# aubin-tchoi/shot-fpfh

Measured on AMD Instinct MI355X. Metric: descriptors/sec (SHOT+FPFH) on 1M-pt cloud, higher is better.
Workload: dtype f64

## Files before the change

### shot_fpfh_amd/csrc/match.h

```cpp
#pragma once
#include <algorithm>
#include <cmath>
#include <cstdlib>
#include <functional>

#include "common.h"

int sf_match_exact(sf_ctx *ctx, const double *da, int64_t m1, const double *db, int64_t m2, int64_t d, int64_t *didx,
                   double *ddist, const char *name, const unsigned char *a_ok, const unsigned char *b_ok);
int sf_match_gemm(sf_ctx *ctx, const double *da, int64_t m1, const double *db, int64_t m2, int64_t d, int64_t *didx,
                  double *ddist, const char *name, int64_t *n_slow, const unsigned char *a_ok, const unsigned char *b_ok);
int sf_match_sqnorm(sf_ctx *ctx, const char *name, const double *rows, int64_t m, int64_t d, const unsigned char *ok, double *out);
int sf_match_gemm_f64(sf_ctx *ctx, const double *da, int64_t m1, const double *db, int64_t m2, int64_t d, int64_t *didx,
                      double *ddist, const char *name, int64_t *n_slow, const unsigned char *a_ok, const unsigned char *b_ok);
int sf_match_half_mode();
int sf_match_half(sf_ctx *ctx, const double *da, int64_t m1, const double *db, int64_t m2, int64_t d, int64_t *didx,
                  double *ddist, const char *name, int64_t *n_slow, const unsigned char *a_ok, const unsigned char *b_ok,
                  int *used);
int sf_match_i8_mode();
int sf_match_i8(sf_ctx *ctx, const double *da, int64_t m1, const double *db, int64_t m2, int64_t d, int64_t *didx,
                double *ddist, const char *name, int64_t *n_slow, const unsigned char *a_ok, const unsigned char *b_ok,
                int *used);

typedef std::function<int(const double *sub, int64_t nr, int64_t *sidx, double *sdist)> sf_match_next;
int sf_match_rescue(sf_ctx *ctx, const double *da, int64_t m1, int64_t d, const int *flag, int nf, const sf_match_next &next,
                    int64_t *didx, double *ddist, int64_t *n_slow, int per_row = 1, const char *gather_name = "k8_gather_rows",
                    const char *scatter_name = "k8_scatter_results");
int sf_match_max(sf_ctx *ctx, const char *name, const double *v, int64_t n, double *part, double *out);

static inline void sf_ransac_band(double thr, double *lo, double *hi)
{
    *lo = *hi = -1.0;
    if (thr >= 0.0) {
        const double up = std::nextafter(thr, INFINITY);
        *lo = std::nextafter(thr * thr, -INFINITY);
        *hi = std::isinf(up) ? INFINITY : std::nextafter(up * up, INFINITY);
        if (std::isinf(thr)) *lo = *hi = INFINITY;
    }
}

static inline bool sf_match_small(int64_t m1, int64_t m2, int64_t d)
{
    return (double)m1 * (double)m2 * (double)d < 5e8 || m2 < 256;
}

static inline int64_t sf_match_col_splits(int64_t row_tiles, int64_t col_tiles, int64_t target, int64_t *tiles_per_split)
{
    int64_t nsplit = 1;
    if (row_tiles < target) nsplit = std::min<int64_t>(col_tiles, sf_div_up(target, row_tiles));
    if (nsplit > 65535) nsplit = 65535;
    *tiles_per_split = sf_div_up(col_tiles, nsplit);
    return sf_div_up(col_tiles, *tiles_per_split);
}

static inline int64_t sf_match_splits(int64_t col_tiles, int64_t tile_bytes, int64_t row_blocks, const char *env)
{
    const int64_t chunk_kb = 8192;
    const int64_t tiles_in_l2 = std::max<int64_t>(8, chunk_kb * 1024 / tile_bytes);
    int64_t nsplit = sf_div_up(col_tiles, tiles_in_l2);
    if (row_blocks * nsplit < 512) nsplit = std::max<int64_t>(nsplit, std::min<int64_t>(sf_div_up(512, row_blocks), std::max<int64_t>(col_tiles / 32, 1)));
    if (const char *e = getenv(env)) nsplit = std::max<int64_t>(1, std::min<int64_t>(atoll(e), col_tiles));
    return nsplit;
}

template <int CTRL>
__device__ __forceinline__ int sf_dpp(int v)
{
    return __builtin_amdgcn_update_dpp(0, v, CTRL, 0xf, 0xf, false);
}
template <int CTRL>
__device__ __forceinline__ float sf_dpp(float v)
{
    return __int_as_float(sf_dpp<CTRL>(__float_as_int(v)));
}
template <int CTRL>
__device__ __forceinline__ double sf_dpp(double v)
{
    return __hiloint2double(sf_dpp<CTRL>(__double2hiint(v)), sf_dpp<CTRL>(__double2loint(v)));
}

__device__ __forceinline__ double sf_match_tol(int64_t d, double na, double nb_max)
{
    return 8.0 * (double)d * 1.1102230246251565e-16 * (na + nb_max);
}

struct sf_recheck {
    double best = INFINITY;
    int64_t bj = -1;
    bool ok = true;
};

__device__ __forceinline__ void sf_recheck_candidate(sf_recheck &r, const double *ai, const double *b, int64_t d, int64_t j,
                                                     double key, double na, double unit, double half_w)
{
    const double *bjp = b + j * d;
    double acc = 0.0;
    for (int64_t u = 0; u < d; ++u) {
        const double df = ai[u] - bjp[u];
        acc += df * df;
    }
    r.ok &= fabs((acc - na) * unit - key) <= half_w;
    const double dj = sqrt(acc);
    if (dj < r.best || (dj == r.best && j < r.bj) || r.bj < 0) {
        if (!(dj == dj)) return;
        r.best = dj;
        r.bj = j;
    }
}

template <int LPR>
__device__ __forceinline__ void sf_recheck_fold(sf_recheck &r)
{
#pragma unroll
    for (int off = LPR / 2; off > 0; off >>= 1) {
        const double ob = __shfl_xor(r.best, off);
        const int64_t oj = __shfl_xor(r.bj, off);
        const int om = __shfl_xor((int)r.ok, off);
        if (oj >= 0 && (r.bj < 0 || ob < r.best || (ob == r.best && oj < r.bj))) {
            r.best = ob;
            r.bj = oj;
        }
        r.ok = r.ok && om;
    }
}
```

### shot_fpfh_amd/csrc/match_half.hip

```cpp
#include <algorithm>
#include <cmath>
#include <cstdlib>

#include "device_util.h"
#include "match.h"

namespace {

typedef _Float16 h8 __attribute__((ext_vector_type(8)));
typedef float f16v __attribute__((ext_vector_type(16)));

constexpr int HM = 256;
constexpr int HN = 64;
constexpr int HCAP = 32;

__global__ __launch_bounds__(256) void k_half_convert(const double *__restrict__ a, int64_t m, int64_t m_pad, int64_t d,
                                                      int dp, double scale, const unsigned char *__restrict__ ok,
                                                      _Float16 *__restrict__ out, double *__restrict__ err,
                                                      double *__restrict__ qn, double *__restrict__ n2,
                                                      float *__restrict__ n2f, double n2f_scale)
{
    const int lane = threadIdx.x & 63;
    const int64_t i = (int64_t)blockIdx.x * 4 + (threadIdx.x >> 6);
    if (i >= m_pad) return;
// ... 154 lines not shown
        f16v acc[2];
        acc[0] = cold ? zero : T;
        acc[1] = acc[0];
#pragma unroll
        for (int ks = 0; ks < KS; ++ks) {
            acc[0] = __builtin_amdgcn_mfma_f32_32x32x16_f16(af[ks], q0[ks % PF], acc[0], 0, 0, 0);
            acc[1] = __builtin_amdgcn_mfma_f32_32x32x16_f16(af[ks], q1[ks % PF], acc[1], 0, 0, 0);
            if (ks + PF < KS) {
                q0[ks % PF] = SF_H_FRAG(ks + PF, 0);
                q1[ks % PF] = SF_H_FRAG(ks + PF, 1);
            }
        }
        __builtin_amdgcn_sched_group_barrier(0x100, 2 * PF, 0);
#pragma unroll
        for (int ks = 0; ks < KS; ++ks) {
            __builtin_amdgcn_sched_group_barrier(0x008, 2, 0);
            if (ks + PF < KS) __builtin_amdgcn_sched_group_barrier(0x100, 2, 0);
        }
        const float *nbl = reinterpret_cast<const float *>(bp + HN * PC * 16);
        const float nbv2[2] = {nbl[r31], nbl[32 + r31]};
#pragma unroll
        for (int cb = 0; cb < 2; ++cb) {
            const int64_t j = jt * HN + 32 * cb + r31;
            const float nbv = nbv2[cb];
            float mx = acc[cb][0];
#pragma unroll
            for (int r = 1; r < 16; ++r) mx = fmaxf(mx, acc[cb][r]);
            if (cold || __ballot(mx >= nbv)) {
                const bool was_cold = cold;
                int rowb = (int)(row0 - rb * HM) + 4 * h;
                asm volatile("" : "+v"(rowb));
                const int64_t rowbase = rb * HM + rowb;
#pragma unroll
                for (int r = 0; r < 16; ++r) {
                    const float dot = was_cold ? acc[cb][r] : acc[cb][r] - T[r];
                    const float key = nbv - dot;
                    const bool hit = (key <= T[r]) & (key < INFINITY);
                    if (__ballot(hit)) {
                        float v = hit ? key : INFINITY;
                        v = fminf(v, sf_dpp<0xB1>(v));
                        v = fminf(v, sf_dpp<0x4E>(v));
                        v = fminf(v, sf_dpp<0x141>(v));
                        v = fminf(v, sf_dpp<0x140>(v));
                        v = fminf(v, __shfl_xor(v, 16));
                        const int64_t row = rowbase + (r & 3) + 8 * (r >> 2);
                        const float tn = fminf(T[r], v + win[row]);
                        if (hit && key <= tn) {
                            const int s = atomicAdd(&cnt[row], 1);
                            if (s < HCAP) {
                                cand_j[row * HCAP + s] = (int32_t)j;
                                cand_k[row * HCAP + s] = key;
                            }
                        }
                        if (cb == 0 && !was_cold) acc[1][r] += tn - T[r];
                        T[r] = tn;
                    }
                }
                if (was_cold && cb == 1) {
                    bool c = false;
#pragma unroll
                    for (int r = 0; r < 16; ++r) c |= T[r] == INFINITY;
                    cold = __ballot(c) != 0;
                }
            }
        }
        asm volatile("s_waitcnt vmcnt(0)" ::: "memory");
        __syncthreads();
    }
    if (r31 == 0) {
#pragma unroll
        for (int r = 0; r < 16; ++r) {
            const int64_t row = row0 + (r & 3) + 8 * (r >> 2) + 4 * h;
            thr_out[row] = T[r];
            if (thr_best && row < m1 && T[r] < INFINITY) atomic_min_f32(thr_best + row, T[r]);
        }
    }
#undef SF_H_DMA
#undef SF_H_DMA16
#undef SF_H_DMA4
#undef SF_H_FRAG
}

template <int LPR>
__global__ void k_half_final(const double *__restrict__ a, int64_t m1, const double *__restrict__ b, int64_t d,
                             const unsigned char *__restrict__ a_ok, const int *__restrict__ cnt,
                             const int32_t *__restrict__ cand_j, const float *__restrict__ cand_k,
                             const float *__restrict__ thr, const float *__restrict__ win,
                             const double *__restrict__ na2, double unit, int nsplit, int64_t m1_pad,
                             int64_t *__restrict__ idx,
                             double *__restrict__ dist, int *__restrict__ flag, int *__restrict__ n_flagged)
{
    const int64_t gid = (int64_t)blockIdx.x * blockDim.x + threadIdx.x;
    const int64_t i = gid / LPR;
    const int sub = (int)(gid % LPR);
    if (i >= m1) return;
    if (a_ok && !a_ok[i]) {
        if (sub == 0) {
            idx[i] = 0;
            if (dist) dist[i] = INFINITY;
            flag[i] = 0;
        }
        return;
    }
    float t = INFINITY;
    for (int s = 0; s < nsplit; ++s) t = fminf(t, thr[(int64_t)s * m1_pad + i]);
    bool overflow = false;
    const float w = win[i] * 1.001f;
    for (int s = 0; s < nsplit; ++s)
        overflow |= cnt[(int64_t)s * m1_pad + i] > HCAP && !(thr[(int64_t)s * m1_pad + i] - w > t);
    sf_recheck r;
    if (!overflow) {
        const double *ai = a + i * d;
        const double half_w = 0.5 * (double)win[i], na = na2[i];
        for (int s = 0; s < nsplit; ++s) {
            const int64_t base = ((int64_t)s * m1_pad + i) * HCAP;
            const int n = min(cnt[(int64_t)s * m1_pad + i], HCAP);
            for (int c = sub; c < n; c += LPR)
                if (cand_k[base + c] <= t)
                    sf_recheck_candidate(r, ai, b, d, cand_j[base + c], (double)cand_k[base + c], na, unit, half_w);
        }
    }
    sf_recheck_fold<LPR>(r);
    if (sub != 0) return;
    const bool decided = r.bj >= 0 && r.ok;
    idx[i] = decided ? r.bj : 0;
    if (dist) dist[i] = r.best;
    flag[i] = decided ? 0 : 1;
    if (!decided) atomicAdd(n_flagged, 1);
}

bool pick_scale(double n2max, double *scale)
{
    if (!(n2max > 0.0) || !std::isfinite(n2max)) return false;
    int e = 0;
    std::frexp(std::sqrt(n2max), &e);
    const int k = 14 - e;
    if (k < -100 || k > 100) return false;
    *scale = std::ldexp(1.0, k);
    return true;
}

}

int sf_match_half_mode()
{
    const char *e = getenv("SF_MATCH_HALF");
    if (!e || !e[0]) return -1;
    return e[0] == '0' ? 0 : 1;
}

int sf_match_half(sf_ctx *ctx, const double *da, int64_t m1, const double *db, int64_t m2, int64_t d, int64_t *didx,
                  double *ddist, const char *name, int64_t *n_slow, const unsigned char *a_ok, const unsigned char *b_ok,
                  int *used)
{
    *used = 0;
    if (d > 352 || m1 <= 0 || m2 <= 0 || m2 > 0x7fffffff) return SF_OK;
    const int ks = d <= 128 ? 8 : 22, dp = 16 * ks;
    const int64_t m1p = sf_div_up(m1, HM) * HM, m2p = sf_div_up(m2, HN) * HN;
    _Float16 *ah = nullptr, *bh = nullptr;
    double *ea = nullptr, *qa = nullptr, *na2 = nullptr, *eb = nullptr, *qb = nullptr, *nb2 = nullptr, *part = nullptr;
    float *nbf = nullptr, *win = nullptr, *candk = nullptr, *thr = nullptr;
    int *cnt = nullptr, *flag = nullptr, *nflag = nullptr;
    int32_t *candj = nullptr;
    sf_pool_guard tmp(ctx);
#define SF_HALLOC(ptr, count) SF_CHECK(tmp.alloc(&ptr, (size_t)(count)))
    SF_HALLOC(part, 256);
    SF_HALLOC(nb2, m2p); SF_HALLOC(eb, m2p); SF_HALLOC(qb, m2p); SF_HALLOC(nbf, m2p);
    SF_HALLOC(na2, m1p); SF_HALLOC(ea, m1p); SF_HALLOC(qa, m1p);
    SF_HALLOC(ah, m1p * dp); SF_HALLOC(bh, m2p * dp);
    double namax = 0.0, nbmax = 0.0, sa = 1.0, sb = 1.0;
    {
        SF_LAUNCH(ctx, "k8_half_convert", k_half_convert, dim3((unsigned)sf_div_up(m1p, 4)), dim3(256), da, m1, m1p, d, dp,
                  1.0, (const unsigned char *)nullptr, (_Float16 *)nullptr, ea, qa, na2, (float *)nullptr, 1.0);
        SF_LAUNCH(ctx, "k8_half_convert", k_half_convert, dim3((unsigned)sf_div_up(m2p, 4)), dim3(256), db, m2, m2p, d, dp,
                  1.0, b_ok, (_Float16 *)nullptr, eb, qb, nb2, (float *)nullptr, 1.0);
        int rc = sf_match_max(ctx, "k8_half_max", na2, m1, part, &namax);
        if (rc == SF_OK) rc = sf_match_max(ctx, "k8_half_max", nb2, m2, part, &nbmax);
        if (rc != SF_OK) return rc;
    }
    if (!pick_scale(namax, &sa) || !pick_scale(nbmax, &sb)) return SF_OK;
    const double unit = 0.5 * sa * sb;
    if (!(nbmax * unit < 1e30) || !(nbmax * unit > 1e-20)) return SF_OK;
    SF_LAUNCH(ctx, "k8_half_convert", k_half_convert, dim3((unsigned)sf_div_up(m1p, 4)), dim3(256), da, m1, m1p, d, dp, sa,
              (const unsigned char *)nullptr, ah, ea, qa, na2, (float *)nullptr, 1.0);
    SF_LAUNCH(ctx, "k8_half_convert", k_half_convert, dim3((unsigned)sf_div_up(m2p, 4)), dim3(256), db, m2, m2p, d, dp, sb,
              b_ok, bh, eb, qb, nb2, nbf, unit);
    double ebmax = 0.0, qbmax = 0.0;
    {
        int rc = sf_match_max(ctx, "k8_half_max", eb, m2, part, &ebmax);
        if (rc == SF_OK) rc = sf_match_max(ctx, "k8_half_max", qb, m2, part, &qbmax);
        if (rc != SF_OK) return rc;
    }
    if (!std::isfinite(ebmax) || !std::isfinite(qbmax)) return SF_OK;
    const int64_t col_tiles = m2p / HN;
    int64_t nsplit = sf_match_splits(col_tiles, (int64_t)HN * dp * 2, m1p / HM, "SF_MATCH_HALF_SPLITS");
    const int64_t tiles_per_split = sf_div_up(col_tiles, nsplit);
    nsplit = sf_div_up(col_tiles, tiles_per_split);
    const bool seed = true;
    const int64_t slab_rows = std::min<int64_t>(m1p, HM * std::max<int64_t>(64, ((int64_t)8 << 30) / (nsplit * HCAP * 8 * HM)));
    float *tbest = nullptr;
    SF_HALLOC(win, slab_rows); SF_HALLOC(thr, nsplit * slab_rows); SF_HALLOC(cnt, nsplit * slab_rows); SF_HALLOC(tbest, slab_rows);
    SF_HALLOC(candj, nsplit * slab_rows * HCAP); SF_HALLOC(candk, nsplit * slab_rows * HCAP);
    SF_HALLOC(flag, m1); SF_HALLOC(nflag, 1);
    const double gamma = (double)(dp + 32) * 2.384185791015625e-07;
    SF_HIP(hipMemsetAsync(nflag, 0, sizeof(int), ctx->stream));
    for (int64_t r0 = 0; r0 < m1; r0 += slab_rows) {
        const int64_t ms = std::min(m1 - r0, slab_rows), msp = sf_div_up(ms, HM) * HM, row_blocks = msp / HM;
        SF_LAUNCH(ctx, "k8_half_window", k_half_window, dim3((unsigned)sf_div_up(msp, 256)), dim3(256), (const double *)(ea + r0),
                  (const double *)(qa + r0), (const double *)(na2 + r0), ms, msp, std::sqrt(nbmax), ebmax, qbmax, nbmax, gamma, unit, win);
        SF_HIP(hipMemsetAsync(cnt, 0, (size_t)(nsplit * msp) * sizeof(int), ctx->stream));
        SF_HIP(hipMemsetD32Async((hipDeviceptr_t)tbest, 0x7f800000, (size_t)msp, ctx->stream));
        const int64_t wgs = sf_xcd_grid(nsplit * row_blocks);
        if (wgs > 0x7fffffffLL) { sf_set_error("sf_match_half: %lld workgroups exceed a launch", (long long)wgs); return SF_ERR_UNSUPPORTED; }
        if (ks == 8) {
            SF_LAUNCH(ctx, name, k_match_half<8>, dim3((unsigned)wgs), dim3(512), (const _Float16 *)(ah + r0 * dp),
                      ms, (const _Float16 *)bh, m2p, (const float *)nbf, (const float *)win, tiles_per_split, msp, row_blocks, nsplit,
                      seed ? tbest : (float *)nullptr, cnt, candj, candk, thr);
        } else {
            SF_LAUNCH(ctx, name, k_match_half<22>, dim3((unsigned)wgs), dim3(512), (const _Float16 *)(ah + r0 * dp),
                      ms, (const _Float16 *)bh, m2p, (const float *)nbf, (const float *)win, tiles_per_split, msp, row_blocks, nsplit,
                      seed ? tbest : (float *)nullptr, cnt, candj, candk, thr);
        }
#define SF_HALF_FINAL(LPR)                                                                                            \
        SF_LAUNCH(ctx, "k8_half_final", k_half_final<LPR>, dim3((unsigned)sf_div_up(ms * LPR, 256)), dim3(256), da + r0 * d, ms, db, d, \
                  a_ok ? a_ok + r0 : a_ok, (const int *)cnt, (const int32_t *)candj, (const float *)candk, (const float *)thr, \
                  (const float *)win, (const double *)(na2 + r0), unit, (int)nsplit, msp, didx + r0, ddist ? ddist + r0 : ddist, \
                  flag + r0, nflag);
        const int lpr = ms <= 160000 ? 16 : 1;
        if (lpr == 1) { SF_HALF_FINAL(1) } else { SF_HALF_FINAL(16) }
#undef SF_HALF_FINAL
    }
    int nf = 0;
    SF_HIP(hipMemcpyAsync(&nf, nflag, sizeof(int), hipMemcpyDeviceToHost, ctx->stream));
    SF_HIP(hipStreamSynchronize(ctx->stream));
    const int rc = sf_match_rescue(ctx, da, m1, d, flag, nf, [&](const double *sub, int64_t nr, int64_t *sidx, double *sdist) {
        return sf_match_gemm_f64(ctx, sub, nr, db, m2, d, sidx, sdist, "k8_match_gemm_overflow", nullptr, nullptr, b_ok);
    }, didx, ddist, n_slow);
#undef SF_HALLOC
    *used = 1;
    return rc;
}
```

### shot_fpfh_amd/csrc/match_i8.hip

```cpp
#include <algorithm>
#include <cmath>
#include <cstdlib>
#include <vector>

#include "device_util.h"
#include "match.h"

namespace {

typedef int i4v __attribute__((ext_vector_type(4)));
typedef int i16v __attribute__((ext_vector_type(16)));

constexpr int IN = 64;
constexpr int ICAP = 32;
constexpr int I_LIVE = 4;
constexpr int I_BIG = 1 << 30;
constexpr int I_REAL = 1 << 29;

__global__ __launch_bounds__(256) void k_i8_rowstat(const double *__restrict__ a, int64_t m, int64_t d, double *__restrict__ n2,
                                                    double *__restrict__ amax)
{
    const int lane = threadIdx.x & 63;
    const int64_t i = (int64_t)blockIdx.x * 4 + (threadIdx.x >> 6);
    if (i >= m) return;
// ... 281 lines not shown
    }
}

template <int KS>
__global__ __launch_bounds__(512, 1) void k_i8_collect(const unsigned char *__restrict__ ai, const unsigned char *__restrict__ bi,
                                                        const int *__restrict__ nbs, const int2 *__restrict__ split_tiles,
                                                        int64_t n_blocks, const int *__restrict__ blk_split,
                                                        const int *__restrict__ pair_row, const int *__restrict__ pair_thr,
                                                        int *__restrict__ cnt, int32_t *__restrict__ cand_j,
                                                        int *__restrict__ cand_k)
{
    const int64_t vb = sf_xcd_block();
    if (vb >= n_blocks) return;
    const int64_t split = blk_split[vb];
    SF_I_GEOMETRY
    const int64_t p0 = vb * 256 + 32 * wave;
    i4v af[KS];
    {
        const int row = pair_row[p0 + r31];
        const unsigned char *ap = ai + (int64_t)(row < 0 ? 0 : row) * DP + 16 * h;
#pragma unroll
        for (int ks = 0; ks < KS; ++ks) af[ks] = *reinterpret_cast<const i4v *>(ap + 32 * ks);
#pragma unroll
        for (int ks = 0; ks < KS; ++ks) asm volatile("" : "+v"(af[ks]));
    }
    i16v T;
#pragma unroll
    for (int r = 0; r < 16; ++r) {
        const int64_t p = p0 + (r & 3) + 8 * (r >> 2) + 4 * h;
        T[r] = pair_row[p] < 0 ? -I_BIG : pair_thr[p];
    }
    const int2 st = split_tiles[split];
    const int64_t jt0 = st.x, ntiles = st.y;
    SF_I_DMA(jt0, 0)
    asm volatile("s_waitcnt vmcnt(0)" ::: "memory");
    __syncthreads();
    for (int64_t jt = jt0; jt < ntiles; ++jt) {
        const int buf = (int)((jt - jt0) & 1);
        if (jt + 1 < ntiles) SF_I_DMA(jt + 1, buf ^ 1)
        const unsigned char *bp = Bs + buf * TILE_BYTES;
        constexpr int PF = 3;
        const int *nbl = reinterpret_cast<const int *>(bp + IN * PC * 16);
#pragma unroll 1
        for (int cb = 0; cb < 2; ++cb) {
            i4v q[PF];
#pragma unroll
            for (int i = 0; i < PF; ++i) q[i] = SF_I_FRAG(i, cb);
            i16v acc = T;
#pragma unroll
            for (int ks = 0; ks < KS; ++ks) {
                acc = __builtin_amdgcn_mfma_i32_32x32x32_i8(af[ks], q[ks % PF], acc, 0, 0, 0);
                if (ks + PF < KS) q[ks % PF] = SF_I_FRAG(ks + PF, cb);
            }
            const int nbv = nbl[32 * cb + r31];
            int mx = acc[0];
#pragma unroll
            for (int r = 1; r < 16; ++r) mx = max(mx, acc[r]);
            if (__ballot(mx >= nbv && nbv < I_REAL)) {
                const int64_t j = jt * IN + 32 * cb + r31;
#pragma unroll
                for (int r = 0; r < 16; ++r) {
                    if (acc[r] >= nbv && nbv < I_REAL) {
                        const int64_t p = p0 + (r & 3) + 8 * (r >> 2) + 4 * h;
                        const int s = atomicAdd(&cnt[p], 1);
                        if (s < ICAP) {
                            cand_j[p * ICAP + s] = (int32_t)j;
                            cand_k[p * ICAP + s] = nbv - (acc[r] - T[r]);
                        }
                    }
                }
            }
        }
        asm volatile("s_waitcnt vmcnt(0)" ::: "memory");
        __syncthreads();
    }
}
#undef SF_I_DMA
#undef SF_I_DMA16
#undef SF_I_DMA4
#undef SF_I_FRAG
#undef SF_I_GEOMETRY

template <int LPR>
__global__ void k_i8_final(const double *__restrict__ a, int64_t m1, const double *__restrict__ b, int64_t d,
                           const unsigned char *__restrict__ a_ok, const int *__restrict__ live, const int *__restrict__ cnt,
                           const int32_t *__restrict__ cand_j, const int *__restrict__ cand_k, const int *__restrict__ win,
                           const double *__restrict__ na2, double unit, int64_t *__restrict__ idx, double *__restrict__ dist,
                           int *__restrict__ flag, int *__restrict__ n_flagged)
{
    const int64_t gid = (int64_t)blockIdx.x * blockDim.x + threadIdx.x;
    const int64_t i = gid / LPR;
    const int sub = (int)(gid % LPR);
    if (i >= m1) return;
    if ((a_ok && !a_ok[i]) || flag[i]) return;
    sf_recheck r;
    const double *ai = a + i * d;
    const double half_w = 0.5 * (double)win[i], na = na2[i];
    for (int l = 0; l < I_LIVE; ++l) {
        const int p = live[i * I_LIVE + l];
        if (p < 0) continue;
        const int n = cnt[p];
        if (n > ICAP) { r.ok = false; continue; }
        const int64_t base = (int64_t)p * ICAP;
        for (int c = sub; c < n; c += LPR)
            sf_recheck_candidate(r, ai, b, d, cand_j[base + c], (double)cand_k[base + c], na, unit, half_w);
    }
    sf_recheck_fold<LPR>(r);
    if (sub != 0) return;
    const bool decided = r.bj >= 0 && r.ok;
    idx[i] = decided ? r.bj : 0;
    if (dist) dist[i] = r.best;
    if (!decided) {
        flag[i] = 1;
        atomicAdd(n_flagged, 1);
    }
}

}

int sf_match_i8_mode()
{
    const char *e = getenv("SF_MATCH_I8");
    if (!e || !e[0]) return -1;
    return e[0] == '0' ? 0 : 1;
}

struct sf_match_stream {
    sf_ctx *ctx = nullptr;
    const double *da = nullptr, *db = nullptr;
    const unsigned char *a_ok = nullptr, *b_ok = nullptr;
    int64_t m1 = 0, m2 = 0, d = 0, m1p = 0, m2p = 0;
    int ks = 11, dp = 352, RB = 2, IM = 512;
    double sa = 0.0, sb = 0.0, unit = 0.0;
    bool integer = false;
    bool windowed = false;
    unsigned char *ai = nullptr, *bi = nullptr;
    double *ea = nullptr, *qa = nullptr, *na2 = nullptr, *eb = nullptr, *qb = nullptr, *nb2 = nullptr, *part = nullptr, *amx = nullptr;
    int *nbi = nullptr, *win = nullptr, *smin = nullptr, *kmin = nullptr, *live = nullptr, *flag = nullptr, *counters = nullptr;
    int2 *split_tiles = nullptr;
    int64_t split_cap = 0, tiles_target = 0;
    std::vector<int2> splits;
    std::vector<void *> owned;
    double nbmax = 0.0, ebmax = 0.0;
};

namespace {

template <typename T>
int st_alloc(sf_match_stream *st, T **p, size_t count)
{
    SF_CHECK(sf_palloc(st->ctx, p, count ? count : 1));
    st->owned.push_back(*p);
    return SF_OK;
}

void st_free(sf_match_stream *st)
{
    if (!st) return;
    for (void *p : st->owned) sf_pool_release(st->ctx, p);
    delete st;
}

int st_begin(sf_match_stream *st, double b_entry_max, int64_t max_ranges, bool *suitable)
{
    sf_ctx *ctx = st->ctx;
    *suitable = false;
    const int64_t m1 = st->m1, m2 = st->m2, d = st->d;
    if (d > 352 || m1 <= 0 || m2 <= 0 || m2 > 0x7fffffff || m1 > 0x3fffffff) return SF_OK;
    st->RB = 2;
    st->IM = 256 * st->RB;
    st->ks = d <= 128 ? 4 : 11;
    st->dp = 32 * st->ks;
    st->m1p = sf_div_up(m1, 512) * 512;
    st->m2p = sf_div_up(m2, IN) * IN;
    const int64_t m1p = st->m1p, m2p = st->m2p;
    SF_CHECK(st_alloc(st, &st->part, 256));
    SF_CHECK(st_alloc(st, &st->na2, m1p)); SF_CHECK(st_alloc(st, &st->ea, m1p)); SF_CHECK(st_alloc(st, &st->qa, m1p));
    SF_CHECK(st_alloc(st, &st->amx, std::max(m1, m2)));
    double namax = 0.0, aamax = 0.0;
    SF_LAUNCH(ctx, "k8_i8_convert", k_i8_rowstat, dim3((unsigned)sf_div_up(m1, 4)), dim3(256), st->da, m1, d, st->na2, st->amx);
    SF_CHECK(sf_match_max(ctx, "k8_i8_max", st->na2, m1, st->part, &namax));
    SF_CHECK(sf_match_max(ctx, "k8_i8_max", st->amx, m1, st->part, &aamax));
    if (!(aamax > 0.0) || !(b_entry_max > 0.0) || !std::isfinite(namax) || !std::isfinite(aamax) || !std::isfinite(b_entry_max)) return SF_OK;
    st->sa = 127.0 / aamax;
    st->sb = 127.0 / b_entry_max;
    st->unit = 0.5 * st->sa * st->sb;
    if (!std::isfinite(st->sa) || !std::isfinite(st->sb) || !std::isfinite(st->unit) || !(st->unit > 0.0)) return SF_OK;
    SF_CHECK(st_alloc(st, &st->ai, m1p * st->dp)); SF_CHECK(st_alloc(st, &st->bi, m2p * st->dp));
    SF_CHECK(st_alloc(st, &st->nb2, m2p)); SF_CHECK(st_alloc(st, &st->eb, m2p)); SF_CHECK(st_alloc(st, &st->qb, m2p)); SF_CHECK(st_alloc(st, &st->nbi, m2p));
    if (m1p > m1) SF_HIP(hipMemsetAsync(st->na2 + m1, 0, (size_t)(m1p - m1) * sizeof(double), ctx->stream));
    SF_LAUNCH(ctx, "k8_i8_convert", k_i8_convert, dim3((unsigned)sf_div_up(m1p, 4)), dim3(256), st->da, m1, m1p, d, st->dp, st->sa,
              (const unsigned char *)nullptr, reinterpret_cast<unsigned *>(st->ai), st->ea, st->qa, (const double *)st->na2, (int *)nullptr, st->unit);
    const int64_t col_tiles = m2p / IN;
    const int64_t nsplit = sf_match_splits(col_tiles, (int64_t)IN * st->dp, m1p / st->IM, "SF_MATCH_I8_SPLITS");
    st->tiles_target = sf_div_up(col_tiles, nsplit);
    st->split_cap = sf_div_up(col_tiles, st->tiles_target) + std::max<int64_t>(max_ranges, 1);
    if (st->split_cap > 65536) return SF_OK;
    SF_CHECK(st_alloc(st, &st->win, m1p)); SF_CHECK(st_alloc(st, &st->smin, st->split_cap * m1p)); SF_CHECK(st_alloc(st, &st->kmin, m1p));
    SF_CHECK(st_alloc(st, &st->live, m1p * I_LIVE)); SF_CHECK(st_alloc(st, &st->flag, m1));
    SF_CHECK(st_alloc(st, &st->counters, 2 * st->split_cap + 2));
    SF_CHECK(st_alloc(st, &st->split_tiles, st->split_cap));
    SF_HIP(hipMemsetAsync(st->counters, 0, (size_t)(2 * st->split_cap + 2) * sizeof(int), ctx->stream));
    *suitable = true;
    st->integer = true;
    return SF_OK;
}

int st_convert_cols(sf_match_stream *st, int64_t rb, int64_t re, int64_t *first, int64_t *count)
{
    sf_ctx *ctx = st->ctx;
    const int64_t rows = re - rb, rows_p = sf_div_up(rows, IN) * IN;
    if (rb % IN || rows <= 0 || re > st->m2 || (re % IN && re != st->m2)) { sf_set_error("sf_match_stream_feed: rows [%lld, %lld) are not whole 64-row tiles", (long long)rb, (long long)re); return SF_ERR_ARG; }
    SF_LAUNCH(ctx, "k8_i8_convert", k_i8_rowstat, dim3((unsigned)sf_div_up(rows, 4)), dim3(256), st->db + rb * st->d, rows, st->d, st->nb2 + rb, st->amx);
    if (rows_p > rows) SF_HIP(hipMemsetAsync(st->nb2 + re, 0, (size_t)(rows_p - rows) * sizeof(double), ctx->stream));
    SF_LAUNCH(ctx, "k8_i8_convert", k_i8_convert, dim3((unsigned)sf_div_up(rows_p, 4)), dim3(256), st->db + rb * st->d, rows, rows_p, st->d, st->dp, st->sb,
              st->b_ok ? st->b_ok + rb : st->b_ok, reinterpret_cast<unsigned *>(st->bi + rb * st->dp), st->eb + rb, st->qb + rb,
              (const double *)(st->nb2 + rb), st->nbi + rb, st->unit);
    const int64_t t0 = rb / IN, t1 = t0 + rows_p / IN, n = sf_div_up(t1 - t0, st->tiles_target), per = sf_div_up(t1 - t0, n);
    *first = (int64_t)st->splits.size();
    for (int64_t t = t0; t < t1; t += per) st->splits.push_back(make_int2((int)t, (int)std::min(t + per, t1)));
    *count = (int64_t)st->splits.size() - *first;
    if ((int64_t)st->splits.size() > st->split_cap) { sf_set_error("sf_match_stream_feed: more ranges than announced"); return SF_ERR_ARG; }
    SF_HIP(hipMemcpyAsync(st->split_tiles + *first, st->splits.data() + *first, (size_t)*count * sizeof(int2), hipMemcpyHostToDevice, ctx->stream));
    SF_HIP(hipStreamSynchronize(ctx->stream));
    return SF_OK;
}

int st_pass1(sf_match_stream *st, const char *name, int64_t first, int64_t count, int64_t r0, int64_t ms)
{
    sf_ctx *ctx = st->ctx;
    const int64_t msp = sf_div_up(ms, st->IM) * st->IM, row_blocks = msp / st->IM;
    const int64_t wgs = sf_xcd_grid(count * row_blocks);
    if (wgs > 0x7fffffffLL) { sf_set_error("sf_match_i8: %lld workgroups exceed a launch", (long long)wgs); return SF_ERR_UNSUPPORTED; }
    if (!count || !ms) return SF_OK;
#define SF_I8_MIN(KS_, RB_)                                                                                             \
    SF_LAUNCH(ctx, name, (k_i8_min<KS_, RB_>), dim3((unsigned)wgs), dim3(512), (const unsigned char *)(st->ai + r0 * st->dp), \
              (const unsigned char *)st->bi, (const int *)st->nbi, (const int2 *)st->split_tiles, first, st->m1p, row_blocks, count, st->smin + r0)
    if (st->ks == 4) { SF_I8_MIN(4, 2); } else { SF_I8_MIN(11, 2); }
#undef SF_I8_MIN
    return SF_OK;
}

int st_window(sf_match_stream *st, bool *suitable)
{
    sf_ctx *ctx = st->ctx;
    *suitable = false;
    SF_CHECK(sf_match_max(ctx, "k8_i8_max", st->nb2, st->m2, st->part, &st->nbmax));
    SF_CHECK(sf_match_max(ctx, "k8_i8_max", st->eb, st->m2, st->part, &st->ebmax));
    if (!std::isfinite(st->nbmax) || !std::isfinite(st->ebmax) || !(st->nbmax * st->unit < 4e6)) return SF_OK;
    SF_LAUNCH(ctx, "k8_i8_window", k_i8_window, dim3((unsigned)sf_div_up(st->m1p, 256)), dim3(256), (const double *)st->ea, (const double *)st->qa,
              (const double *)st->na2, st->m1, st->m1p, std::sqrt(st->nbmax), st->ebmax, st->nbmax, st->unit, st->win);
    st->windowed = true;
    *suitable = true;
    return SF_OK;
}

int st_decide(sf_match_stream *st, int64_t r0, int64_t ms, int64_t *didx, double *ddist)
{
    sf_ctx *ctx = st->ctx;
    const int64_t nsplit = (int64_t)st->splits.size(), m1p = st->m1p;
    int *nflag = st->counters, *split_count = st->counters + 2, *split_cursor = st->counters + 2 + st->split_cap;
    SF_HIP(hipMemsetAsync(split_count, 0, (size_t)(2 * st->split_cap) * sizeof(int), ctx->stream));
    SF_LAUNCH(ctx, "k8_i8_live", k_i8_live, dim3((unsigned)sf_div_up(ms, 256)), dim3(256), (const int *)(st->smin + r0), (const int *)(st->win + r0),
              st->a_ok ? st->a_ok + r0 : st->a_ok, ms, m1p, (int)nsplit, st->kmin + r0, st->live + r0 * I_LIVE, split_count, didx + r0,
              ddist ? ddist + r0 : ddist, st->flag + r0, nflag);
    std::vector<int> hcount((size_t)nsplit), hbase((size_t)nsplit), hblk;
    SF_HIP(hipMemcpyAsync(hcount.data(), split_count, (size_t)nsplit * sizeof(int), hipMemcpyDeviceToHost, ctx->stream));
    SF_HIP(hipStreamSynchronize(ctx->stream));
    int64_t n_pairs_pad = 0;
    for (int64_t s = 0; s < nsplit; ++s) {
        hbase[(size_t)s] = (int)n_pairs_pad;
        const int64_t nb = sf_div_up(hcount[(size_t)s], 256);
        for (int64_t k = 0; k < nb; ++k) hblk.push_back((int)s);
        n_pairs_pad += nb * 256;
        if (n_pairs_pad > 0x7fffff00LL) { sf_set_error("sf_match_i8: too many (row, split) pairs"); return SF_ERR_UNSUPPORTED; }
    }
    const int64_t n_blocks = (int64_t)hblk.size();
    sf_pool_guard ptmp(ctx);
    int *split_base = nullptr, *blk_split = nullptr, *pair_row = nullptr, *pair_thr = nullptr, *cnt = nullptr, *candk = nullptr;
    int32_t *candj = nullptr;
    const size_t np1 = (size_t)std::max<int64_t>(n_pairs_pad, 1);
    SF_CHECK(ptmp.alloc(&split_base, (size_t)nsplit)); SF_CHECK(ptmp.alloc(&blk_split, (size_t)std::max<int64_t>(n_blocks, 1)));
    SF_CHECK(ptmp.alloc(&pair_row, np1)); SF_CHECK(ptmp.alloc(&pair_thr, np1)); SF_CHECK(ptmp.alloc(&cnt, np1));
    SF_CHECK(ptmp.alloc(&candj, np1 * ICAP)); SF_CHECK(ptmp.alloc(&candk, np1 * ICAP));
    SF_HIP(hipMemcpyAsync(split_base, hbase.data(), (size_t)nsplit * sizeof(int), hipMemcpyHostToDevice, ctx->stream));
    if (n_blocks) {
        SF_HIP(hipMemcpyAsync(blk_split, hblk.data(), (size_t)n_blocks * sizeof(int), hipMemcpyHostToDevice, ctx->stream));
        SF_HIP(hipMemsetAsync(pair_row, 0xff, (size_t)n_pairs_pad * sizeof(int), ctx->stream));
        SF_HIP(hipMemsetAsync(cnt, 0, (size_t)n_pairs_pad * sizeof(int), ctx->stream));
        SF_LAUNCH(ctx, "k8_i8_live", k_i8_place, dim3((unsigned)sf_div_up(ms, 256)), dim3(256), (const int *)(st->kmin + r0), (const int *)(st->win + r0),
                  st->live + r0 * I_LIVE, ms, (int)nsplit, (const int *)split_base, split_cursor, pair_row, pair_thr);
        const int64_t cw = sf_xcd_grid(n_blocks);
        if (st->ks == 4) {
            SF_LAUNCH(ctx, "k8_i8_collect", k_i8_collect<4>, dim3((unsigned)cw), dim3(512), (const unsigned char *)(st->ai + r0 * st->dp),
                      (const unsigned char *)st->bi, (const int *)st->nbi, (const int2 *)st->split_tiles, n_blocks, (const int *)blk_split,
                      (const int *)pair_row, (const int *)pair_thr, cnt, candj, candk);
        } else {
            SF_LAUNCH(ctx, "k8_i8_collect", k_i8_collect<11>, dim3((unsigned)cw), dim3(512), (const unsigned char *)(st->ai + r0 * st->dp),
                      (const unsigned char *)st->bi, (const int *)st->nbi, (const int2 *)st->split_tiles, n_blocks, (const int *)blk_split,
                      (const int *)pair_row, (const int *)pair_thr, cnt, candj, candk);
        }
    }
#define SF_I8_FINAL(LPR)                                                                                               \
    SF_LAUNCH(ctx, "k8_i8_final", k_i8_final<LPR>, dim3((unsigned)sf_div_up(ms * LPR, 256)), dim3(256), st->da + r0 * st->d, ms, st->db, st->d, \
              st->a_ok ? st->a_ok + r0 : st->a_ok, (const int *)(st->live + r0 * I_LIVE), (const int *)cnt, (const int32_t *)candj, \
              (const int *)candk, (const int *)(st->win + r0), (const double *)(st->na2 + r0), st->unit, didx + r0,          \
              ddist ? ddist + r0 : ddist, st->flag + r0, nflag)
    if (ms <= 65536) { SF_I8_FINAL(16); } else { SF_I8_FINAL(1); }
#undef SF_I8_FINAL
    SF_HIP(hipStreamSynchronize(ctx->stream));
    return SF_OK;
}

int st_flagged(sf_match_stream *st, int *nf)
{
    SF_HIP(hipMemcpyAsync(nf, st->counters, sizeof(int), hipMemcpyDeviceToHost, st->ctx->stream));
    SF_HIP(hipStreamSynchronize(st->ctx->stream));
    return SF_OK;
}

int st_fallback(sf_match_stream *st, int nf, int64_t *didx, double *ddist, int64_t *n_slow)
{
    return sf_match_rescue(st->ctx, st->da, st->m1, st->d, st->flag, nf, [st](const double *sub, int64_t nr, int64_t *sidx, double *sdist) {
        int used = 0;
        int rc = sf_match_half(st->ctx, sub, nr, st->db, st->m2, st->d, sidx, sdist, "k8_match_half", nullptr, nullptr, st->b_ok, &used);
        if (rc == SF_OK && !used)
            rc = sf_match_gemm_f64(st->ctx, sub, nr, st->db, st->m2, st->d, sidx, sdist, "k8_match_gemm_overflow", nullptr, nullptr, st->b_ok);
        return rc;
    }, didx, ddist, n_slow);
}

}

int sf_match_i8(sf_ctx *ctx, const double *da, int64_t m1, const double *db, int64_t m2, int64_t d, int64_t *didx, double *ddist,
                const char *name, int64_t *n_slow, const unsigned char *a_ok, const unsigned char *b_ok, int *used)
{
    *used = 0;
    if (d > 352 || m1 <= 0 || m2 <= 0 || m2 > 0x7fffffff || m1 > 0x3fffffff) return SF_OK;
    sf_match_stream *st = new sf_match_stream();
    st->ctx = ctx; st->da = da; st->db = db; st->a_ok = a_ok; st->b_ok = b_ok; st->m1 = m1; st->m2 = m2; st->d = d;
    struct guard { sf_match_stream *s; ~guard() { st_free(s); } } g{st};
    double abmax = 0.0;
    {
        sf_pool_guard tmp(ctx);
        double *n2 = nullptr, *mx = nullptr, *part = nullptr;
        SF_CHECK(tmp.alloc(&n2, (size_t)m2)); SF_CHECK(tmp.alloc(&mx, (size_t)m2)); SF_CHECK(tmp.alloc(&part, 256));
        SF_LAUNCH(ctx, "k8_i8_convert", k_i8_rowstat, dim3((unsigned)sf_div_up(m2, 4)), dim3(256), db, m2, d, n2, mx);
        SF_CHECK(sf_match_max(ctx, "k8_i8_max", mx, m2, part, &abmax));
    }
    bool ok = false;
    SF_CHECK(st_begin(st, abmax, 1, &ok));
    if (!ok) return SF_OK;
    int64_t first = 0, count = 0;
    SF_CHECK(st_convert_cols(st, 0, m2, &first, &count));
    SF_CHECK(st_window(st, &ok));
    if (!ok) return SF_OK;
    static const double max_flagged = [] { const char *e = getenv("SF_I8_MAX_FLAGGED"); const double v = e ? atof(e) : 0.35; return v > 0.0 ? v : 0.35; }();
    const char *pilot_env = getenv("SF_I8_PILOT_ROWS");
    const int64_t pilot_rows = pilot_env ? std::max<int64_t>(st->IM, sf_div_up(atoll(pilot_env), st->IM) * st->IM) : (int64_t)st->IM * 64;
    const bool pilot = pilot_env ? m1 > pilot_rows : (m1 >= 4 * pilot_rows && sf_match_i8_mode() != 1);
    int64_t done = 0;
    int nf = 0;
    if (pilot) {
        SF_CHECK(st_pass1(st, name, first, count, 0, pilot_rows));
        SF_CHECK(st_decide(st, 0, pilot_rows, didx, ddist));
        SF_CHECK(st_flagged(st, &nf));
        if ((double)nf > max_flagged * (double)pilot_rows) return SF_OK;
        done = pilot_rows;
    }
    SF_CHECK(st_pass1(st, name, first, count, done, m1 - done));
    SF_CHECK(st_decide(st, done, m1 - done, didx, ddist));
    SF_CHECK(st_flagged(st, &nf));
    const int rc = st_fallback(st, nf, didx, ddist, n_slow);
    *used = 1;
    return rc;
}

extern "C" sf_match_stream *sf_match_stream_begin(sf_ctx *ctx, const double *a_dev, const unsigned char *a_ok_dev, int64_t m1,
                                                  const double *b_dev, const unsigned char *b_ok_dev, int64_t m2, int64_t d,
                                                  double b_entry_max, int64_t max_ranges)
{
    if (!ctx || !a_dev || !b_dev || !a_ok_dev || !b_ok_dev || m1 < 0 || m2 <= 0 || d <= 0) { sf_set_error("sf_match_stream_begin: bad argument"); return nullptr; }
    if (hipSetDevice(ctx->device) != hipSuccess) { sf_set_error("hipSetDevice failed"); return nullptr; }
    sf_match_stream *st = new sf_match_stream();
    st->ctx = ctx; st->da = a_dev; st->db = b_dev; st->a_ok = a_ok_dev; st->b_ok = b_ok_dev; st->m1 = m1; st->m2 = m2; st->d = d;
    bool ok = false;
    const bool wanted = sf_match_i8_mode() != 0 && m1 > 0;
    if (wanted && st_begin(st, b_entry_max, max_ranges, &ok) != SF_OK) { st_free(st); return nullptr; }
    return st;
}

extern "C" int sf_match_stream_feed(sf_ctx *ctx, sf_match_stream *st, int64_t row_begin, int64_t row_end)
{
    if (!ctx || !st || st->ctx != ctx) { sf_set_error("sf_match_stream_feed: bad argument"); return SF_ERR_ARG; }
    if (!st->integer) return SF_OK;
    SF_HIP(hipSetDevice(ctx->device));
    int64_t first = 0, count = 0;
    SF_CHECK(st_convert_cols(st, row_begin, row_end, &first, &count));
    return st_pass1(st, "k8_match_i8", first, count, 0, st->m1);
}

extern "C" int sf_match_stream_end(sf_ctx *ctx, sf_match_stream *st, int64_t *idx_dev, double *dist_dev)
{
    if (!ctx || !st || st->ctx != ctx || !idx_dev) { sf_set_error("sf_match_stream_end: bad argument"); return SF_ERR_ARG; }
    struct guard { sf_match_stream *s; ~guard() { st_free(s); } } g{st};
    SF_HIP(hipSetDevice(ctx->device));
    if (st->integer) {
        int64_t tiles = 0;
        for (const int2 &sp : st->splits) tiles += sp.y - sp.x;
        if (tiles != st->m2p / IN) { sf_set_error("sf_match_stream_end: %lld of %lld column tiles were fed", (long long)tiles, (long long)(st->m2p / IN)); return SF_ERR_STATE; }
        bool ok = false;
        SF_CHECK(st_window(st, &ok));
        if (ok) {
            static const double max_flagged = [] { const char *e = getenv("SF_I8_MAX_FLAGGED"); const double v = e ? atof(e) : 0.35; return v > 0.0 ? v : 0.35; }();
            int nf = 0;
            SF_CHECK(st_decide(st, 0, st->m1, idx_dev, dist_dev));
            SF_CHECK(st_flagged(st, &nf));
            if ((double)nf <= max_flagged * (double)st->m1 || sf_match_i8_mode() == 1) return st_fallback(st, nf, idx_dev, dist_dev, nullptr);
        }
    }
    return sf_match_argmin_multiscale(ctx, st->da, st->db, 1, st->m1, st->m2, st->d, st->a_ok, st->b_ok, INFINITY, idx_dev, dist_dev,
                                      SF_IN_DEVICE | SF_OUT_DEVICE);
}

extern "C" void sf_match_stream_abort(sf_ctx *ctx, sf_match_stream *st)
{
    (void)ctx;
    st_free(st);
}
```

Baseline: 556.7 million.

## Stage candidate recheck rows through LDS and reuse precomputed B norms

```diff
diff --git a/shot_fpfh_amd/csrc/match.h b/shot_fpfh_amd/csrc/match.h
--- a/shot_fpfh_amd/csrc/match.h
+++ b/shot_fpfh_amd/csrc/match.h
@@ -16,7 +16,7 @@
 int sf_match_half_mode();
 int sf_match_half(sf_ctx *ctx, const double *da, int64_t m1, const double *db, int64_t m2, int64_t d, int64_t *didx,
                   double *ddist, const char *name, int64_t *n_slow, const unsigned char *a_ok, const unsigned char *b_ok,
-                  int *used);
+                  int *used, const double *nb2_max = nullptr);
 int sf_match_i8_mode();
 int sf_match_i8(sf_ctx *ctx, const double *da, int64_t m1, const double *db, int64_t m2, int64_t d, int64_t *didx,
                 double *ddist, const char *name, int64_t *n_slow, const unsigned char *a_ok, const unsigned char *b_ok,
@@ -90,15 +90,9 @@
     bool ok = true;
 };
 
-__device__ __forceinline__ void sf_recheck_candidate(sf_recheck &r, const double *ai, const double *b, int64_t d, int64_t j,
-                                                     double key, double na, double unit, double half_w)
+__device__ __forceinline__ void sf_recheck_update(sf_recheck &r, double acc, int64_t j, double key, double na, double unit,
+                                                  double half_w)
 {
-    const double *bjp = b + j * d;
-    double acc = 0.0;
-    for (int64_t u = 0; u < d; ++u) {
-        const double df = ai[u] - bjp[u];
-        acc += df * df;
-    }
     r.ok &= fabs((acc - na) * unit - key) <= half_w;
     const double dj = sqrt(acc);
     if (dj < r.best || (dj == r.best && j < r.bj) || r.bj < 0) {
@@ -106,6 +100,85 @@
         r.best = dj;
         r.bj = j;
     }
+}
+
+constexpr int SF_RC_CHUNK = 32;
+constexpr int SF_RC_STRIDE = SF_RC_CHUNK + 1;
+
+template <int LPR>
+struct sf_recheck_lds {
+    static_assert(LPR == 1 || LPR == 2 || LPR == 4 || LPR == 8 || LPR == 16, "the rows of a wave come in groups of four");
+    static constexpr int SCAN = 64 / LPR, ROWS = SCAN + 64, LOADS = ROWS / 4;
+    double img[ROWS * SF_RC_STRIDE];
+    long long row[ROWS];
+};
+
+template <int LPR>
+__device__ __forceinline__ void sf_recheck_round(sf_recheck &r, sf_recheck_lds<LPR> &sh, const double *a, int64_t i, const double *b,
+                                                 int64_t d, bool have, int64_t j, double key, double na, double unit,
+                                                 double half_w)
+{
+    typedef sf_recheck_lds<LPR> L;
+    const int lane = threadIdx.x & 63;
+    const unsigned long long mask = __ballot(have);
+    const bool group_has = ((mask >> (lane / LPR * LPR)) & ((1ull << LPR) - 1ull)) != 0;
+    const long long a_first = (long long)(i * d), b_first = (long long)((have ? j : 0) * d);
+    if (lane % LPR == 0) sh.row[lane / LPR] = group_has ? a_first : -1ll;
+    sh.row[L::SCAN + lane] = have ? b_first : -1ll;
+    const long long a_par = (long long)((size_t)a >> 3), b_par = (long long)((size_t)b >> 3);
+    const int pa = (int)((a_par + a_first) & 1), pb = (int)((b_par + b_first) & 1);
+    const bool shifted = __ballot(have && (pa | pb)) != 0;
+    const int64_t npos = d + (shifted ? 1 : 0);
+    const int nchunk = (int)((npos + SF_RC_CHUNK - 1) / SF_RC_CHUNK);
+    const int lo = pa > pb ? pa : pb;
+    const int64_t hi = d + lo;
+    __syncthreads();
+    const int lrow = lane >> 4, lpos = 2 * (lane & 15);
+    long long first[L::LOADS];
+#pragma unroll
+    for (int t = 0; t < L::LOADS; ++t) first[t] = sh.row[4 * t + lrow];
+    double2 v[L::LOADS];
+    auto load = [&](int k) {
+#pragma unroll
+        for (int t = 0; t < L::LOADS; ++t) {
+            const bool scan = 4 * t < L::SCAN;
+            v[t] = make_double2(0.0, 0.0);
+            if (first[t] >= 0) {
+                const int par = (int)(((scan ? a_par : b_par) + first[t]) & 1);
+                const int64_t p0 = (int64_t)k * SF_RC_CHUNK + lpos;
+                const double *src = (scan ? a : b) + (first[t] - par) + p0;
+                const bool x_in = p0 >= par && p0 < d + par, y_in = p0 + 1 < d + par;
+                if (x_in && y_in) v[t] = *reinterpret_cast<const double2 *>(src);
+                else if (x_in) v[t].x = src[0];
+                else if (y_in) v[t].y = src[1];
+            }
+        }
+    };
+    double acc = 0.0, a_prev = 0.0, b_prev = 0.0;
+    const double *ia = sh.img + (lane / LPR) * SF_RC_STRIDE, *ib = sh.img + (L::SCAN + lane) * SF_RC_STRIDE;
+    load(0);
+    for (int k = 0; k < nchunk; ++k) {
+#pragma unroll
+        for (int t = 0; t < L::LOADS; ++t) {
+            double *dst = sh.img + (4 * t + lrow) * SF_RC_STRIDE + lpos;
+            dst[0] = v[t].x;
+            dst[1] = v[t].y;
+        }
+        __syncthreads();
+        if (k + 1 < nchunk) load(k + 1);
+        const int64_t p0 = (int64_t)k * SF_RC_CHUNK;
+#pragma unroll
+        for (int t = 0; t < SF_RC_CHUNK; ++t) {
+            const double x = ia[t], y = ib[t];
+            const double df = (pa < pb ? a_prev : x) - (pb < pa ? b_prev : y);
+            a_prev = x;
+            b_prev = y;
+            const double next = acc + df * df;
+            acc = (p0 + t >= lo && p0 + t < hi) ? next : acc;
+        }
+        __syncthreads();
+    }
+    if (have) sf_recheck_update(r, acc, j, key, na, unit, half_w);
 }
 
 template <int LPR>
diff --git a/shot_fpfh_amd/csrc/match_half.hip b/shot_fpfh_amd/csrc/match_half.hip
--- a/shot_fpfh_amd/csrc/match_half.hip
+++ b/shot_fpfh_amd/csrc/match_half.hip
@@ -260,7 +260,7 @@
 }
 
 template <int LPR>
-__global__ void k_half_final(const double *__restrict__ a, int64_t m1, const double *__restrict__ b, int64_t d,
+__global__ __launch_bounds__(64) void k_half_final(const double *__restrict__ a, int64_t m1, const double *__restrict__ b, int64_t d,
                              const unsigned char *__restrict__ a_ok, const int *__restrict__ cnt,
                              const int32_t *__restrict__ cand_j, const float *__restrict__ cand_k,
                              const float *__restrict__ thr, const float *__restrict__ win,
@@ -268,38 +268,52 @@
                              int64_t *__restrict__ idx,
                              double *__restrict__ dist, int *__restrict__ flag, int *__restrict__ n_flagged)
 {
+    __shared__ sf_recheck_lds<LPR> sh;
     const int64_t gid = (int64_t)blockIdx.x * blockDim.x + threadIdx.x;
     const int64_t i = gid / LPR;
     const int sub = (int)(gid % LPR);
-    if (i >= m1) return;
-    if (a_ok && !a_ok[i]) {
-        if (sub == 0) {
-            idx[i] = 0;
-            if (dist) dist[i] = INFINITY;
-            flag[i] = 0;
-        }
-        return;
-    }
+    const bool real = i < m1;
+    const bool masked = real && a_ok && !a_ok[i];
+    if (masked && sub == 0) {
+        idx[i] = 0;
+        if (dist) dist[i] = INFINITY;
+        flag[i] = 0;
+    }
+    const bool mine = real && !masked;
     float t = INFINITY;
-    for (int s = 0; s < nsplit; ++s) t = fminf(t, thr[(int64_t)s * m1_pad + i]);
     bool overflow = false;
-    const float w = win[i] * 1.001f;
-    for (int s = 0; s < nsplit; ++s)
-        overflow |= cnt[(int64_t)s * m1_pad + i] > HCAP && !(thr[(int64_t)s * m1_pad + i] - w > t);
+    if (mine) {
+        for (int s = 0; s < nsplit; ++s) t = fminf(t, thr[(int64_t)s * m1_pad + i]);
+        const float w = win[i] * 1.001f;
+        for (int s = 0; s < nsplit; ++s)
+            overflow |= cnt[(int64_t)s * m1_pad + i] > HCAP && !(thr[(int64_t)s * m1_pad + i] - w > t);
+    }
     sf_recheck r;
-    if (!overflow) {
-        const double *ai = a + i * d;
-        const double half_w = 0.5 * (double)win[i], na = na2[i];
-        for (int s = 0; s < nsplit; ++s) {
-            const int64_t base = ((int64_t)s * m1_pad + i) * HCAP;
-            const int n = min(cnt[(int64_t)s * m1_pad + i], HCAP);
-            for (int c = sub; c < n; c += LPR)
-                if (cand_k[base + c] <= t)
-                    sf_recheck_candidate(r, ai, b, d, cand_j[base + c], (double)cand_k[base + c], na, unit, half_w);
-        }
+    const double half_w = mine ? 0.5 * (double)win[i] : 0.0, na = mine ? na2[i] : 0.0;
+    int s = (mine && !overflow) ? 0 : nsplit, c = 0, n = 0;
+    int64_t base = 0;
+    for (;;) {
+        for (;;) {
+            if (c >= n) {
+                if (s >= nsplit) break;
+                base = ((int64_t)s * m1_pad + i) * HCAP;
+                n = min(cnt[(int64_t)s * m1_pad + i], HCAP);
+                c = sub;
+                ++s;
+            } else if (cand_k[base + c] <= t) {
+                break;
+            } else {
+                c += LPR;
+            }
+        }
+        const bool have = c < n;
+        if (!__ballot(have)) break;
+        sf_recheck_round<LPR>(r, sh, a, mine ? i : 0, b, d, have, have ? (int64_t)cand_j[base + c] : 0, have ? (double)cand_k[base + c] : 0.0, na,
+                              unit, half_w);
+        c += LPR;
     }
     sf_recheck_fold<LPR>(r);
-    if (sub != 0) return;
+    if (!mine || sub != 0) return;
     const bool decided = r.bj >= 0 && r.ok;
     idx[i] = decided ? r.bj : 0;
     if (dist) dist[i] = r.best;
@@ -329,7 +343,7 @@
 
 int sf_match_half(sf_ctx *ctx, const double *da, int64_t m1, const double *db, int64_t m2, int64_t d, int64_t *didx,
                   double *ddist, const char *name, int64_t *n_slow, const unsigned char *a_ok, const unsigned char *b_ok,
-                  int *used)
+                  int *used, const double *nb2_max)
 {
     *used = 0;
     if (d > 352 || m1 <= 0 || m2 <= 0 || m2 > 0x7fffffff) return SF_OK;
@@ -350,10 +364,14 @@
     {
         SF_LAUNCH(ctx, "k8_half_convert", k_half_convert, dim3((unsigned)sf_div_up(m1p, 4)), dim3(256), da, m1, m1p, d, dp,
                   1.0, (const unsigned char *)nullptr, (_Float16 *)nullptr, ea, qa, na2, (float *)nullptr, 1.0);
-        SF_LAUNCH(ctx, "k8_half_convert", k_half_convert, dim3((unsigned)sf_div_up(m2p, 4)), dim3(256), db, m2, m2p, d, dp,
-                  1.0, b_ok, (_Float16 *)nullptr, eb, qb, nb2, (float *)nullptr, 1.0);
         int rc = sf_match_max(ctx, "k8_half_max", na2, m1, part, &namax);
-        if (rc == SF_OK) rc = sf_match_max(ctx, "k8_half_max", nb2, m2, part, &nbmax);
+        if (nb2_max) {
+            nbmax = *nb2_max;
+        } else {
+            SF_LAUNCH(ctx, "k8_half_convert", k_half_convert, dim3((unsigned)sf_div_up(m2p, 4)), dim3(256), db, m2, m2p, d, dp,
+                      1.0, b_ok, (_Float16 *)nullptr, eb, qb, nb2, (float *)nullptr, 1.0);
+            if (rc == SF_OK) rc = sf_match_max(ctx, "k8_half_max", nb2, m2, part, &nbmax);
+        }
         if (rc != SF_OK) return rc;
     }
     if (!pick_scale(namax, &sa) || !pick_scale(nbmax, &sb)) return SF_OK;
@@ -400,7 +418,7 @@
                       seed ? tbest : (float *)nullptr, cnt, candj, candk, thr);
         }
 #define SF_HALF_FINAL(LPR)                                                                                            \
-        SF_LAUNCH(ctx, "k8_half_final", k_half_final<LPR>, dim3((unsigned)sf_div_up(ms * LPR, 256)), dim3(256), da + r0 * d, ms, db, d, \
+        SF_LAUNCH(ctx, "k8_half_final", k_half_final<LPR>, dim3((unsigned)sf_div_up(ms * LPR, 64)), dim3(64), da + r0 * d, ms, db, d, \
                   a_ok ? a_ok + r0 : a_ok, (const int *)cnt, (const int32_t *)candj, (const float *)candk, (const float *)thr, \
                   (const float *)win, (const double *)(na2 + r0), unit, (int)nsplit, msp, didx + r0, ddist ? ddist + r0 : ddist, \
                   flag + r0, nflag);
diff --git a/shot_fpfh_amd/csrc/match_i8.hip b/shot_fpfh_amd/csrc/match_i8.hip
--- a/shot_fpfh_amd/csrc/match_i8.hip
+++ b/shot_fpfh_amd/csrc/match_i8.hip
@@ -387,31 +387,38 @@
 #undef SF_I_GEOMETRY
 
 template <int LPR>
-__global__ void k_i8_final(const double *__restrict__ a, int64_t m1, const double *__restrict__ b, int64_t d,
+__global__ __launch_bounds__(64) void k_i8_final(const double *__restrict__ a, int64_t m1, const double *__restrict__ b, int64_t d,
                            const unsigned char *__restrict__ a_ok, const int *__restrict__ live, const int *__restrict__ cnt,
                            const int32_t *__restrict__ cand_j, const int *__restrict__ cand_k, const int *__restrict__ win,
                            const double *__restrict__ na2, double unit, int64_t *__restrict__ idx, double *__restrict__ dist,
                            int *__restrict__ flag, int *__restrict__ n_flagged)
 {
+    __shared__ sf_recheck_lds<LPR> sh;
     const int64_t gid = (int64_t)blockIdx.x * blockDim.x + threadIdx.x;
     const int64_t i = gid / LPR;
     const int sub = (int)(gid % LPR);
-    if (i >= m1) return;
-    if ((a_ok && !a_ok[i]) || flag[i]) return;
+    const bool mine = i < m1 && !(a_ok && !a_ok[i]) && !flag[i];
     sf_recheck r;
-    const double *ai = a + i * d;
-    const double half_w = 0.5 * (double)win[i], na = na2[i];
-    for (int l = 0; l < I_LIVE; ++l) {
-        const int p = live[i * I_LIVE + l];
-        if (p < 0) continue;
-        const int n = cnt[p];
-        if (n > ICAP) { r.ok = false; continue; }
-        const int64_t base = (int64_t)p * ICAP;
-        for (int c = sub; c < n; c += LPR)
-            sf_recheck_candidate(r, ai, b, d, cand_j[base + c], (double)cand_k[base + c], na, unit, half_w);
+    const double half_w = mine ? 0.5 * (double)win[i] : 0.0, na = mine ? na2[i] : 0.0;
+    int l = mine ? 0 : I_LIVE, c = 0, n = 0;
+    int64_t base = 0;
+    for (;;) {
+        while (c >= n && l < I_LIVE) {
+            const int p = live[i * I_LIVE + l++];
+            if (p < 0) continue;
+            n = cnt[p];
+            if (n > ICAP) { r.ok = false; n = 0; continue; }
+            base = (int64_t)p * ICAP;
+            c = sub;
+        }
+        const bool have = c < n;
+        if (!__ballot(have)) break;
+        sf_recheck_round<LPR>(r, sh, a, mine ? i : 0, b, d, have, have ? (int64_t)cand_j[base + c] : 0, have ? (double)cand_k[base + c] : 0.0, na,
+                              unit, half_w);
+        c += LPR;
     }
     sf_recheck_fold<LPR>(r);
-    if (sub != 0) return;
+    if (!mine || sub != 0) return;
     const bool decided = r.bj >= 0 && r.ok;
     idx[i] = decided ? r.bj : 0;
     if (dist) dist[i] = r.best;
@@ -447,6 +454,7 @@
     std::vector<int2> splits;
     std::vector<void *> owned;
     double nbmax = 0.0, ebmax = 0.0;
+    const double *nb2_known = nullptr;
 };
 
 namespace {
@@ -516,7 +524,8 @@
     sf_ctx *ctx = st->ctx;
     const int64_t rows = re - rb, rows_p = sf_div_up(rows, IN) * IN;
     if (rb % IN || rows <= 0 || re > st->m2 || (re % IN && re != st->m2)) { sf_set_error("sf_match_stream_feed: rows [%lld, %lld) are not whole 64-row tiles", (long long)rb, (long long)re); return SF_ERR_ARG; }
-    SF_LAUNCH(ctx, "k8_i8_convert", k_i8_rowstat, dim3((unsigned)sf_div_up(rows, 4)), dim3(256), st->db + rb * st->d, rows, st->d, st->nb2 + rb, st->amx);
+    if (st->nb2_known) SF_HIP(hipMemcpyAsync(st->nb2 + rb, st->nb2_known + rb, (size_t)rows * sizeof(double), hipMemcpyDeviceToDevice, ctx->stream));
+    else SF_LAUNCH(ctx, "k8_i8_convert", k_i8_rowstat, dim3((unsigned)sf_div_up(rows, 4)), dim3(256), st->db + rb * st->d, rows, st->d, st->nb2 + rb, st->amx);
     if (rows_p > rows) SF_HIP(hipMemsetAsync(st->nb2 + re, 0, (size_t)(rows_p - rows) * sizeof(double), ctx->stream));
     SF_LAUNCH(ctx, "k8_i8_convert", k_i8_convert, dim3((unsigned)sf_div_up(rows_p, 4)), dim3(256), st->db + rb * st->d, rows, rows_p, st->d, st->dp, st->sb,
               st->b_ok ? st->b_ok + rb : st->b_ok, reinterpret_cast<unsigned *>(st->bi + rb * st->dp), st->eb + rb, st->qb + rb,
@@ -607,7 +616,7 @@
         }
     }
 #define SF_I8_FINAL(LPR)                                                                                               \
-    SF_LAUNCH(ctx, "k8_i8_final", k_i8_final<LPR>, dim3((unsigned)sf_div_up(ms * LPR, 256)), dim3(256), st->da + r0 * st->d, ms, st->db, st->d, \
+    SF_LAUNCH(ctx, "k8_i8_final", k_i8_final<LPR>, dim3((unsigned)sf_div_up(ms * LPR, 64)), dim3(64), st->da + r0 * st->d, ms, st->db, st->d, \
               st->a_ok ? st->a_ok + r0 : st->a_ok, (const int *)(st->live + r0 * I_LIVE), (const int *)cnt, (const int32_t *)candj, \
               (const int *)candk, (const int *)(st->win + r0), (const double *)(st->na2 + r0), st->unit, didx + r0,          \
               ddist ? ddist + r0 : ddist, st->flag + r0, nflag)
@@ -628,7 +637,8 @@
 {
     return sf_match_rescue(st->ctx, st->da, st->m1, st->d, st->flag, nf, [st](const double *sub, int64_t nr, int64_t *sidx, double *sdist) {
         int used = 0;
-        int rc = sf_match_half(st->ctx, sub, nr, st->db, st->m2, st->d, sidx, sdist, "k8_match_half", nullptr, nullptr, st->b_ok, &used);
+        int rc = sf_match_half(st->ctx, sub, nr, st->db, st->m2, st->d, sidx, sdist, "k8_match_half", nullptr, nullptr, st->b_ok, &used,
+                               st->windowed ? &st->nbmax : nullptr);
         if (rc == SF_OK && !used)
             rc = sf_match_gemm_f64(st->ctx, sub, nr, st->db, st->m2, st->d, sidx, sdist, "k8_match_gemm_overflow", nullptr, nullptr, st->b_ok);
         return rc;
@@ -646,12 +656,14 @@
     st->ctx = ctx; st->da = da; st->db = db; st->a_ok = a_ok; st->b_ok = b_ok; st->m1 = m1; st->m2 = m2; st->d = d;
     struct guard { sf_match_stream *s; ~guard() { st_free(s); } } g{st};
     double abmax = 0.0;
+    sf_pool_guard keep(ctx);
     {
         sf_pool_guard tmp(ctx);
         double *n2 = nullptr, *mx = nullptr, *part = nullptr;
-        SF_CHECK(tmp.alloc(&n2, (size_t)m2)); SF_CHECK(tmp.alloc(&mx, (size_t)m2)); SF_CHECK(tmp.alloc(&part, 256));
+        SF_CHECK(keep.alloc(&n2, (size_t)m2)); SF_CHECK(tmp.alloc(&mx, (size_t)m2)); SF_CHECK(tmp.alloc(&part, 256));
         SF_LAUNCH(ctx, "k8_i8_convert", k_i8_rowstat, dim3((unsigned)sf_div_up(m2, 4)), dim3(256), db, m2, d, n2, mx);
         SF_CHECK(sf_match_max(ctx, "k8_i8_max", mx, m2, part, &abmax));
+        st->nb2_known = n2;
     }
     bool ok = false;
     SF_CHECK(st_begin(st, abmax, 1, &ok));
```

Result: no change. 556.5 million (median of 2 runs) (-0.0%).
